# asmirnou/watsor

Measured on NVIDIA H100. Metric: aggregate detection FPS on synthetic 640x480 streams, higher is better.
Workload: dtype f32

## Files before the change

### watsor_b200/csrc/kernels_fused.cu

```cuda
#include <algorithm>
#include <cstdlib>
#include <cstring>

#include "kernels_tc.cuh"
#include "tc_common.cuh"

namespace {

constexpr int F_TH = 8, F_TW = 16;

__device__ __forceinline__ void tma_load_4d(uint32_t dst, const CUtensorMap* map, uint32_t bar, int c0, int c1, int c2,
                                            int c3) {
  asm volatile(
      "cp.async.bulk.tensor.4d.shared::cluster.global.mbarrier::complete_tx::bytes [%0], [%1, {%3, %4, %5, %6}], [%2];" ::
          "r"(dst),
      "l"(map), "r"(bar), "r"(c0), "r"(c1), "r"(c2), "r"(c3)
      : "memory");
}

struct FusedArgs {
  const float* dw_w;
  const float* dw_scale;
  const float* dw_offset;
  const float* scale;
  const float* offset;
  float* out;
  int dw_act, act;
  int C, S, pad_t, pad_l;
  int OH, OW, n_img;
  int N, n_pad, block_n, k_blocks;
  int tiles_x, tiles_y;
  int stages, halo_stages;
  int th_in, tw_in;
};

constexpr int F_CONSUMER_WARPS = 8;
constexpr int F_PRODUCER_WARPS = 8;
constexpr int F_FIRST_PRODUCER_THREAD = 32 * F_CONSUMER_WARPS;
constexpr int F_TMA_WARP = F_CONSUMER_WARPS + F_PRODUCER_WARPS;
constexpr int F_THREADS = F_FIRST_PRODUCER_THREAD + 32 * F_PRODUCER_WARPS + 32;

__device__ __forceinline__ void f_wg_bar_sync(int wg) { asm volatile("bar.sync %0, 128;" ::"r"(2 + wg) : "memory"); }

template <int S, int BN>
__global__ void __launch_bounds__(F_THREADS, 1)
    k_dwpw_tc_x3(const __grid_constant__ CUtensorMap map_in, const __grid_constant__ CUtensorMap map_b,
                 const __grid_constant__ CUtensorMap map_b_lo, FusedArgs g) {
  extern __shared__ __align__(1024) uint8_t smem_raw[];
  uint8_t* smem = reinterpret_cast<uint8_t*>((reinterpret_cast<uintptr_t>(smem_raw) + 1023) & ~(uintptr_t)1023);
  const int halo_bytes = ((g.th_in * g.tw_in * ROW_BYTES + 1023) / 1024) * 1024;
  constexpr int B_TILE_BYTES = BN * ROW_BYTES;
  constexpr int AB_BYTES = 2 * A_TILE_BYTES + 2 * B_TILE_BYTES;
  uint8_t* halo0 = smem;
  uint8_t* ab0 = halo0 + (size_t)g.halo_stages * halo_bytes;
  uint64_t* halo_full = reinterpret_cast<uint64_t*>(ab0 + (size_t)g.stages * AB_BYTES);
  uint64_t* halo_empty = halo_full + g.halo_stages;
  uint64_t* b_full = halo_empty + g.halo_stages;
  uint64_t* a_ready = b_full + g.stages;
  uint64_t* empty = a_ready + g.stages;
  float* s_dw = reinterpret_cast<float*>((reinterpret_cast<uintptr_t>(empty + g.stages) + 15) & ~(uintptr_t)15);

  const int warp = threadIdx.x >> 5, lane = threadIdx.x & 31;
  const int tiles_per_img = g.tiles_x * g.tiles_y;
  const int num_tiles = tiles_per_img * g.n_img;

  if (threadIdx.x == 0) {
    for (int h = 0; h < g.halo_stages; ++h) {
      mbar_init(smem_u32(&halo_full[h]), 1);
      mbar_init(smem_u32(&halo_empty[h]), F_PRODUCER_WARPS);
    }
    for (int s = 0; s < g.stages; ++s) {
      mbar_init(smem_u32(&b_full[s]), 1);
      mbar_init(smem_u32(&a_ready[s]), F_PRODUCER_WARPS);
      mbar_init(smem_u32(&empty[s]), 2);
    }
    fence_barrier_init();
  }
  for (int i = threadIdx.x; i < 9 * g.C; i += blockDim.x) s_dw[i] = g.dw_w[i];
  for (int i = threadIdx.x; i < g.C; i += blockDim.x) {
    s_dw[9 * g.C + i] = g.dw_scale[i];
    s_dw[10 * g.C + i] = g.dw_offset[i];
  }
  float* s_pw = s_dw + 11 * g.C;
  for (int i = threadIdx.x; i < BN; i += blockDim.x) {
    s_pw[i] = i < g.n_pad ? g.scale[i] : 1.f;
    s_pw[BN + i] = i < g.n_pad ? g.offset[i] : 0.f;
  }
  __syncthreads();

  if (warp == F_TMA_WARP) {
    if (elect_one()) {
      int it = 0;
      for (int t = blockIdx.x; t < num_tiles; t += gridDim.x) {
        const int img = t / tiles_per_img, r = t - img * tiles_per_img;
        const int oy0 = (r / g.tiles_x) * F_TH, ox0 = (r % g.tiles_x) * F_TW;
        for (int kb = 0; kb < g.k_blocks; ++kb, ++it) {
          const int h = it % g.halo_stages, s = it % g.stages;
          mbar_wait(smem_u32(&halo_empty[h]), ((it / g.halo_stages) & 1) ^ 1);
          const uint32_t hb = smem_u32(&halo_full[h]);
          mbar_expect_tx(hb, (uint32_t)(g.th_in * g.tw_in * ROW_BYTES));
          tma_load_4d(smem_u32(halo0 + (size_t)h * halo_bytes), &map_in, hb, kb * 32, ox0 * S - g.pad_l,
                      oy0 * S - g.pad_t, img);
          mbar_wait(smem_u32(&empty[s]), ((it / g.stages) & 1) ^ 1);
          const uint32_t bb = smem_u32(&b_full[s]);
          uint8_t* sb = ab0 + (size_t)s * AB_BYTES + 2 * A_TILE_BYTES;
          mbar_expect_tx(bb, 2 * B_TILE_BYTES);
          tma_load_2d(smem_u32(sb), &map_b, bb, kb * 32, 0);
          tma_load_2d(smem_u32(sb + B_TILE_BYTES), &map_b_lo, bb, kb * 32, 0);
        }
      }
    }
  } else if (warp < F_CONSUMER_WARPS) {
    const int wg = warp >> 2;
    const int row = wg * 64 + (warp & 3) * 16 + (lane >> 2);
    const int col = 2 * (lane & 3);
    int it = 0;
    for (int t = blockIdx.x; t < num_tiles; t += gridDim.x) {
      const int img = t / tiles_per_img, r = t - img * tiles_per_img;
      const int oy0 = (r / g.tiles_x) * F_TH, ox0 = (r % g.tiles_x) * F_TW;
      float acc[BN / 2], part[BN / 2];
#pragma unroll
      for (int i = 0; i < BN / 2; ++i) acc[i] = 0.f;
      for (int kb = 0; kb < g.k_blocks; ++kb, ++it) {
        const int s = it % g.stages;
        const uint32_t ph = (it / g.stages) & 1;
        mbar_wait(smem_u32(&a_ready[s]), ph);
        mbar_wait(smem_u32(&b_full[s]), ph);
        const uint32_t a_hi = smem_u32(ab0 + (size_t)s * AB_BYTES) + (uint32_t)(wg * 64 * ROW_BYTES);
        const uint32_t a_lo = a_hi + A_TILE_BYTES;
        const uint32_t b_hi = smem_u32(ab0 + (size_t)s * AB_BYTES) + 2 * A_TILE_BYTES, b_lo = b_hi + B_TILE_BYTES;
        wg_x3_kblock_sum<BN>(acc, part, a_hi, a_lo, b_hi, b_lo);
        f_wg_bar_sync(wg);
        if ((threadIdx.x & 127) == 0) mbar_arrive(smem_u32(&empty[s]));
      }
#pragma unroll
      for (int h = 0; h < 2; ++h) {
        const int rr = row + 8 * h;
        const int oy = oy0 + rr / F_TW, ox = ox0 + rr % F_TW;
        if (oy >= g.OH || ox >= g.OW) continue;
        float* op = g.out + (((size_t)img * g.OH + oy) * g.OW + ox) * g.N;
#pragma unroll
        for (int j = 0; j < BN / 8; ++j) {
          const int c = 8 * j + col;
          if (c >= g.N) break;
          float y0 = affine_rn(acc[4 * j + 2 * h], s_pw[c], s_pw[BN + c]);
          float y1 = affine_rn(acc[4 * j + 2 * h + 1], s_pw[c + 1], s_pw[BN + c + 1]);
          if (g.act == WB_ACT_RELU6) {
            y0 = relu6f(y0);
            y1 = relu6f(y1);
          }
          *reinterpret_cast<float2*>(op + c) = make_float2(y0, y1);
        }
      }
    }
  } else {
    const int pt = threadIdx.x - F_FIRST_PRODUCER_THREAD;
    const int q = pt & 7, slot = pt >> 3;
    int it = 0;
    for (int t = blockIdx.x; t < num_tiles; t += gridDim.x) {
      for (int kb = 0; kb < g.k_blocks; ++kb, ++it) {
        const int h = it % g.halo_stages, s = it % g.stages;
        const int cch = kb * 32 + q * 4;
        float4 wr[9];
#pragma unroll
        for (int k = 0; k < 9; ++k) wr[k] = lds128(smem_u32(s_dw + k * g.C + cch));
        const float4 sc = lds128(smem_u32(s_dw + 9 * g.C + cch));
        const float4 of = lds128(smem_u32(s_dw + 10 * g.C + cch));
        mbar_wait(smem_u32(&halo_full[h]), (it / g.halo_stages) & 1);
        mbar_wait(smem_u32(&empty[s]), ((it / g.stages) & 1) ^ 1);
        const uint32_t hal = smem_u32(halo0 + (size_t)h * halo_bytes);
        const uint32_t a_hi = smem_u32(ab0 + (size_t)s * AB_BYTES);
        const uint32_t a_lo = a_hi + A_TILE_BYTES;
        static_assert(S == 1 && F_PRODUCER_WARPS == 8 && F_TW == 16 && F_TH == 8, "producer mapping");
        constexpr int TW_IN = F_TW + 2;
        const int ty = slot >> 2, x0 = (slot & 3) * 4;
        const uint32_t win = hal + (uint32_t)((ty * TW_IN + x0) * 128 + q * 16);
        float4 acc[4];
#pragma unroll
        for (int o = 0; o < 4; ++o) acc[o] = make_float4(0.f, 0.f, 0.f, 0.f);
#pragma unroll
        for (int ky = 0; ky < 3; ++ky)
#pragma unroll
          for (int c = 0; c < 6; ++c) {
            const float4 x = lds128(win + (uint32_t)((ky * TW_IN + c) * 128));
#pragma unroll
            for (int kx = 0; kx < 3; ++kx) {
              const int o = c - kx;
              if (o >= 0 && o < 4) {
                const float4 ww = wr[ky * 3 + kx];
                acc[o].x = fmaf(x.x, ww.x, acc[o].x);
                acc[o].y = fmaf(x.y, ww.y, acc[o].y);
                acc[o].z = fmaf(x.z, ww.z, acc[o].z);
                acc[o].w = fmaf(x.w, ww.w, acc[o].w);
              }
            }
          }
#pragma unroll
        for (int o = 0; o < 4; ++o) {
          const int r = ty * F_TW + x0 + o;
          float v[4] = {affine_rn(acc[o].x, sc.x, of.x), affine_rn(acc[o].y, sc.y, of.y),
                        affine_rn(acc[o].z, sc.z, of.z), affine_rn(acc[o].w, sc.w, of.w)};
          uint4 hi, lo;
          uint32_t* hp = &hi.x;
          uint32_t* lp = &lo.x;
#pragma unroll
          for (int e = 0; e < 4; ++e) {
            const float a = g.dw_act == WB_ACT_RELU6 ? relu6f(v[e]) : v[e];
            const uint32_t hb = __float_as_uint(a) & 0xFFFFE000u;
            hp[e] = hb;
            lp[e] = __float_as_uint(__fsub_rn(a, __uint_as_float(hb))) & 0xFFFFE000u;
          }
          const uint32_t off = (uint32_t)r * 128u + (uint32_t)((q ^ (r & 7)) << 4);
          sts128(a_hi + off, hi);
          sts128(a_lo + off, lo);
        }
        fence_proxy_async();
        __syncwarp();
        if (lane == 0) {
          mbar_arrive(smem_u32(&a_ready[s]));
          mbar_arrive(smem_u32(&halo_empty[h]));
        }
      }
    }
  }
}

struct FusedPlan {
  int block_n, stages, halo_stages, th_in, tw_in, tiles_x, tiles_y;
  size_t smem;
};

bool make_plan(const wb_layer& dw, const wb_layer& pw, FusedPlan* p) {
  p->block_n = pw.n_pad <= 32 ? 32 : 64;
  p->th_in = (F_TH - 1) * dw.stride + 3;
  p->tw_in = (F_TW - 1) * dw.stride + 3;
  p->tiles_x = (dw.out_w + F_TW - 1) / F_TW;
  p->tiles_y = (dw.out_h + F_TH - 1) / F_TH;
  const size_t halo = ((size_t)p->th_in * p->tw_in * ROW_BYTES + 1023) / 1024 * 1024;
  const size_t ab = 2 * A_TILE_BYTES + 2 * (size_t)p->block_n * ROW_BYTES;
  const size_t budget = 224 * 1024 - 44 * (size_t)dw.out_c;
  for (int st = 2; st >= 1; --st)
    for (int hs = 3; hs >= 2; --hs) {
      if (hs * halo + st * ab <= budget) {
        p->stages = st;
        p->halo_stages = hs;
        p->smem = hs * halo + st * ab + 1024 + 8 * (2 * hs + 3 * st) + 16 + 44 * (size_t)dw.out_c + 8 * (size_t)p->block_n;
        return true;
      }
    }
  return false;
}


}

bool fused_dwpw_supported(const TcWeights& tw, int pw_layer_index, const wb_layer& dw, const wb_layer& pw, int n) {
  if (tw.mode != TC_TF32X3 || getenv("WB_NO_FUSE") != nullptr) return false;
  if (dw.op != WB_OP_DW || pw.op != WB_OP_PW) return false;
  if (dw.kh != 3 || dw.kw != 3 || dw.stride != 1) return false;
  if (dw.out_c % 32 != 0 || pw.in_c != dw.out_c || pw.n_pad > 64 || pw.out_c % 4 != 0) return false;
  {
    const unsigned long long a0 = dw.in_off, a1 = a0 + (unsigned long long)dw.in_h * dw.in_w * dw.in_c;
    const unsigned long long b0 = pw.out_off, b1 = b0 + (unsigned long long)pw.out_h * pw.out_w * pw.out_c;
    if (a0 < b1 && b0 < a1) return false;
  }
  if (!tw.layers[pw_layer_index].ready) return false;
  FusedPlan p;
  if (!make_plan(dw, pw, &p)) return false;
  int dev = 0, sms = 0;
  cudaGetDevice(&dev);
  cudaDeviceGetAttribute(&sms, cudaDevAttrMultiProcessorCount, dev);
  return (long)p.tiles_x * p.tiles_y * n >= sms;
}

int fused_launch_dwpw(const LaunchCtx& lc, const TcWeights& tw, int pw_layer_index, int n, const wb_layer& dw,
                      const wb_layer& pw, const void* in, const float* dw_w, const float* dw_scale, const float* dw_offset,
                      const float* scale, const float* offset, void* out, std::string* err) {
  const TcLayerWeights& w = tw.layers[pw_layer_index];
  FusedPlan p;
  if (!make_plan(dw, pw, &p)) {
    *err = "fused depthwise+pointwise: no shared-memory plan";
    return 1;
  }
  FusedArgs g;
  g.dw_w = dw_w;
  g.dw_scale = dw_scale;
  g.dw_offset = dw_offset;
  g.scale = scale;
  g.offset = offset;
  g.dw_act = dw.act;
  g.act = pw.act;
  g.C = dw.out_c;
  g.S = dw.stride;
  g.pad_t = dw.pad_t;
  g.pad_l = dw.pad_l;
  g.OH = dw.out_h;
  g.OW = dw.out_w;
  g.n_img = n;
  g.N = pw.out_c;
  g.n_pad = pw.n_pad;
  g.block_n = p.block_n;
  g.k_blocks = (dw.out_c + 31) / 32;
  g.out = static_cast<float*>(out);
  g.tiles_x = p.tiles_x;
  g.tiles_y = p.tiles_y;
  g.stages = p.stages;
  g.halo_stages = p.halo_stages;
  g.th_in = p.th_in;
  g.tw_in = p.tw_in;
  alignas(64) CUtensorMap map_in, map_b, map_b_lo;
  {
    unsigned long long dims[4] = {(unsigned long long)dw.in_c, dw.in_w, dw.in_h, (unsigned long long)n};
    unsigned long long st[3] = {(unsigned long long)dw.in_c * 4, (unsigned long long)dw.in_w * dw.in_c * 4,
                                (unsigned long long)dw.in_h * dw.in_w * dw.in_c * 4};
    unsigned box[4] = {32, (unsigned)p.tw_in, (unsigned)p.th_in, 1};
    if (!tc_encode_map(&map_in, in, 4, 4, dims, st, box, false, err)) return 1;
  }
  {
    unsigned long long dims[2] = {(unsigned long long)w.k, (unsigned long long)w.n_pad};
    unsigned long long st[1] = {(unsigned long long)w.k * 4};
    unsigned box[2] = {32, (unsigned)p.block_n};
    if (!tc_encode_map(&map_b, w.w, 4, 2, dims, st, box, true, err)) return 1;
    if (!tc_encode_map(&map_b_lo, w.w_lo, 4, 2, dims, st, box, true, err)) return 1;
  }
  static PerDeviceFlag attr_done[2];
  static int ctas = 0;
  if (ctas == 0) {
    int dev = 0;
    cudaGetDevice(&dev);
    cudaDeviceGetAttribute(&ctas, cudaDevAttrMultiProcessorCount, dev);
  }
  const long tiles = (long)p.tiles_x * p.tiles_y * n;
  const dim3 grid((unsigned)std::min<long>(tiles, ctas));
  auto launch = [&](auto kern, PerDeviceFlag& done) {
    if (!done.get()) {
      cudaError_t e = cudaFuncSetAttribute(kern, cudaFuncAttributeMaxDynamicSharedMemorySize, 227 * 1024);
      if (e != cudaSuccess) return e;
      done.set();
    }
    kern<<<grid, F_THREADS, p.smem, lc.stream>>>(map_in, map_b, map_b_lo, g);
    return cudaGetLastError();
  };
  const cudaError_t e = p.block_n == 32 ? launch(k_dwpw_tc_x3<1, 32>, attr_done[0]) : launch(k_dwpw_tc_x3<1, 64>, attr_done[1]);
  if (e != cudaSuccess) {
    *err = std::string("fused depthwise+pointwise launch: ") + cudaGetErrorString(e);
    return 1;
  }
  ++*lc.launch_counter;
  return 0;
}
```

### watsor_b200/csrc/kernels_tc.cuh

```cuda
#pragma once
#include <string>
#include <vector>

#include "common.cuh"

enum TcMode { TC_BF16 = 0, TC_TF32X1 = 1, TC_TF32X3 = 2 };

struct TcLayerWeights {
  void* w = nullptr;
  void* w_lo = nullptr;
  int n_pad = 0, k = 0, block_n = 0;
  bool ready = false;
  alignas(64) unsigned char tmap_b[128];
  alignas(64) unsigned char tmap_b_lo[128];
};

struct TcWeights {
  int mode = TC_BF16;
  std::vector<TcLayerWeights> layers;
};

bool tc_layer_supported(const wb_layer& L);
int tc_prepare_weights(const std::vector<wb_layer>& layers, const std::vector<wb_tensor_entry>& tensors,
                       const float* host_data, int mode, TcWeights* out, std::string* err);
void tc_free_weights(TcWeights* w);
int tc_launch_gemm(const LaunchCtx& lc, const TcWeights& tw, int layer_index, int n, const wb_layer& L, const void* in,
                   const float* scale, const float* offset, void* out, float* enc, float* logits, int num_anchors,
                   int num_classes_p1, float* partial, size_t partial_floats, int* tile_counters, const void* residual,
                   std::string* err);

bool tc_encode_map(void* map, const void* base, int elem_bytes, int rank, const unsigned long long* dims,
                   const unsigned long long* strides_bytes, const unsigned* box, bool swizzle128, std::string* err,
                   const unsigned* elem_strides = nullptr);

bool fused_dwpw_supported(const TcWeights& tw, int pw_layer_index, const wb_layer& dw, const wb_layer& pw, int n);
int fused_launch_dwpw(const LaunchCtx& lc, const TcWeights& tw, int pw_layer_index, int n, const wb_layer& dw,
                      const wb_layer& pw, const void* in, const float* dw_w, const float* dw_scale, const float* dw_offset,
                      const float* scale, const float* offset, void* out, std::string* err);
```

### watsor_b200/csrc/wb_api.cu

```cuda
#include <dlfcn.h>
#include <nccl.h>

#include <cstdio>
#include <cstdlib>
#include <cstring>
#include <memory>
#include <mutex>
#include <string>
#include <vector>

#include "common.cuh"
#include "kernels_tc.cuh"

#define WB_MAX_CAMERAS 256
#define WB_SLOTS 6

static thread_local std::string g_err;
static int fail(const std::string& msg) {
  g_err = msg;
  return 1;
}
#define CK(call)                                                                              \
  do {                                                                                        \
    cudaError_t e_ = (call);                                                                  \
// ... 293 lines not shown

int wb_set_camera(wb_ctx* c, int cam, int width, int height, int n_zones, const uint8_t* raster, int n_filters,
                  const wb_class_filter* filters, uint32_t cam_flags) {
  REQUIRE(c, "NULL ctx");
  REQUIRE(cam >= 0 && cam < WB_MAX_CAMERAS, "cam_id out of range (0..255)");
  REQUIRE(width > 0 && height > 0, "bad frame size");
  REQUIRE(n_zones >= 0 && n_zones <= WB_MAX_CAMERA_ZONES, "a mask may hold at most 32 zones");
  REQUIRE(n_zones == 0 || raster != nullptr, "zone_raster is NULL");
  REQUIRE(n_filters == 0 || filters != nullptr, "filters is NULL");
  std::lock_guard<std::mutex> lock(c->mu);
  CK(cudaSetDevice(c->device));
  CK(cudaDeviceSynchronize());
  CameraCfg cfg;
  memset(&cfg, 0, sizeof(cfg));
  cfg.width = width;
  cfg.height = height;
  c->max_src_w = std::max(c->max_src_w, width);
  cfg.n_zones = n_zones;
  cfg.has_mask = raster != nullptr ? 1 : 0;
  cfg.check_label = (cam_flags & WB_CAM_NO_LABEL_CHECK) ? 0 : 1;
  for (int i = 0; i < n_filters; ++i) {
    const wb_class_filter& f = filters[i];
    if (f.label == -1) {
      cfg.default_present = 1;
      cfg.default_conf = f.confidence;
      cfg.default_area = f.area;
      cfg.default_has_zone_list = f.has_zone_list ? 1 : 0;
      cfg.default_zone_bits = f.zone_bits;
      continue;
    }
    REQUIRE(f.label >= 0 && f.label < WB_MAX_LABELS, "filter label out of range (0..127)");
    cfg.present[f.label] = 1;
    cfg.conf[f.label] = f.confidence;
    cfg.area[f.label] = f.area;
    cfg.has_zone_list[f.label] = f.has_zone_list ? 1 : 0;
    cfg.zone_bits[f.label] = f.zone_bits;
  }
  if (c->cam_sat[cam]) {
    CK(cudaFree(c->cam_sat[cam]));
    c->cam_sat[cam] = nullptr;
  }
  if (n_zones > 0) {
    size_t sat_elems = (size_t)n_zones * (height + 1) * (width + 1);
    CK(cudaMalloc(&c->cam_sat[cam], sat_elems * sizeof(int32_t)));
    uint8_t* d_r = nullptr;
    size_t rb = (size_t)n_zones * height * width;
    CK(cudaMalloc(&d_r, rb));
    CK(cudaMemcpy(d_r, raster, rb, cudaMemcpyHostToDevice));
    int lcnt = 0;
    LaunchCtx lc{c->slots[0].stream, &lcnt};
    launch_build_sat(lc, d_r, n_zones, height, width, c->cam_sat[cam]);
    CK(cudaGetLastError());
    CK(cudaStreamSynchronize(c->slots[0].stream));
    CK(cudaFree(d_r));
    cfg.sat = c->cam_sat[cam];
  }
  c->h_cams[cam] = cfg;
  CK(cudaMemcpy(c->d_cams + cam, &cfg, sizeof(cfg), cudaMemcpyHostToDevice));
  return 0;
}

int wb_register_host(wb_ctx* c, void* ptr, size_t bytes) {
  REQUIRE(c && ptr && bytes, "NULL argument");
  std::lock_guard<std::mutex> lock(c->mu);
  CK(cudaSetDevice(c->device));
  CK(cudaHostRegister(ptr, bytes, cudaHostRegisterDefault));
  c->registered.push_back(ptr);
  return 0;
}
int wb_unregister_host(wb_ctx* c, void* ptr) {
  REQUIRE(c && ptr, "NULL argument");
  std::lock_guard<std::mutex> lock(c->mu);
  for (size_t i = 0; i < c->registered.size(); ++i)
    if (c->registered[i] == ptr) {
      CK(cudaHostUnregister(ptr));
      c->registered.erase(c->registered.begin() + i);
      return 0;
    }
  return fail("pointer was not registered");
}

}

template <typename T>
static int run_layers(wb_ctx* c, Slot& s, cudaStream_t st, int n, const float* pre, int first_layer,
                      int last_layer) {
  LaunchCtx lc{st, &s.launches};
  T* arena = static_cast<T*>(s.arena);
  const int NA = c->hdr.num_anchors, C1 = c->hdr.num_classes + 1;
  const size_t end = last_layer < 0 ? c->layers.size() : (size_t)last_layer + 1;
  for (size_t li = (size_t)first_layer; li < end; ++li) {
    const wb_layer& L = c->layers[li];
    const T* in = arena + (size_t)L.in_off * n;
    const T* in2 = arena + (size_t)L.in2_off * n;
    T* outp = arena + (size_t)L.out_off * n;
    const float* w = L.w_tensor >= 0 ? c->tensor(L.w_tensor) : nullptr;
    const float* sc = L.scale_tensor >= 0 ? c->tensor(L.scale_tensor) : nullptr;
    const float* of = L.offset_tensor >= 0 ? c->tensor(L.offset_tensor) : nullptr;
    switch (L.op) {
      case WB_OP_STEM:
        launch_stem<T>(lc, s.d_desc, pre, n, L, c->hdr.input_h, c->hdr.input_w, c->hdr.pre_mul, c->hdr.pre_sub, w,
                       sc, of, outp, c->max_src_w);
        break;
      case WB_OP_DW: {
        if (c->precision == 2 && li + 1 < end) {
          const wb_layer& P = c->layers[li + 1];
          if (P.in_off == L.out_off && fused_dwpw_supported(c->tc, (int)li + 1, L, P, n)) {
            std::string err;
            if (fused_launch_dwpw(lc, c->tc, (int)li + 1, n, L, P, static_cast<const void*>(in), w, sc, of,
                                  c->tensor(P.scale_tensor), c->tensor(P.offset_tensor),
                                  static_cast<void*>(arena + (size_t)P.out_off * n), &err))
              return fail("layers " + std::string(L.name) + " + " + P.name + ": " + err);
            ++li;
            break;
          }
        }
        launch_dw<T>(lc, n, L, in, w, sc, of, outp);
        break;
      }
      case WB_OP_ADD:
        launch_add<T>(lc, (size_t)n * L.out_h * L.out_w * L.out_c, in, in2, outp);
        break;
      case WB_OP_MAXPOOL:
      case WB_OP_AVGPOOL:
        launch_pool<T>(lc, n, L, in, outp);
        break;
      case WB_OP_COPY:
        launch_copy_channels<T>(lc, n, L, in, outp);
        break;
      case WB_OP_PW:
      case WB_OP_CONV:
      case WB_OP_HEAD:
        if (c->precision != 0 && tc_layer_supported(L)) {
          const void* residual = nullptr;
          void* dst = static_cast<void*>(outp);
          bool fuse_add = false;
          if (c->precision != 1 && L.op == WB_OP_PW && L.act == WB_ACT_NONE && li + 1 < end && getenv("WB_NO_FUSE_ADD") == nullptr) {
            const wb_layer& A = c->layers[li + 1];
            const unsigned long long a0 = L.in_off, a1 = a0 + (unsigned long long)L.in_h * L.in_w * L.in_c;
            const unsigned long long b0 = A.out_off, b1 = b0 + (unsigned long long)A.out_h * A.out_w * A.out_c;
            if (A.op == WB_OP_ADD && (A.in_off == L.out_off || A.in2_off == L.out_off) && A.in_off != A.in2_off &&
                !(a0 < b1 && b0 < a1)) {
              const uint32_t other = A.in_off == L.out_off ? A.in2_off : A.in_off;
              residual = static_cast<const void*>(arena + (size_t)other * n);
              dst = static_cast<void*>(arena + (size_t)A.out_off * n);
              fuse_add = true;
            }
          }
          std::string err;
          if (tc_launch_gemm(lc, c->tc, (int)li, n, L, static_cast<const void*>(in), sc, of, dst, s.d_enc, s.d_logits, NA,
                             C1, s.d_partial, s.partial_floats, s.d_tile_counters, residual, &err))
            return fail("layer " + std::string(L.name) + ": " + err);
          if (fuse_add) ++li;
        } else {
          launch_gemm_cc<T>(lc, n, L, in, w, sc, of, outp, s.d_enc, s.d_logits, NA, C1, s.d_partial, s.partial_floats);
        }
        break;
      default:
        return fail("unknown layer op " + std::to_string(L.op));
    }
  }
  CK(cudaGetLastError());
  return 0;
}

static int run_post(wb_ctx* c, Slot& s, cudaStream_t st, int n, uint32_t flags, bool want_raw = false) {
  LaunchCtx lc{st, &s.launches};
  float* rb = want_raw ? s.d_raw : nullptr;
  float* rs = want_raw ? rb + (size_t)c->max_batch * WB_MAX_DETECTIONS * 4 : nullptr;
  float* rc = want_raw ? rs + (size_t)c->max_batch * WB_MAX_DETECTIONS : nullptr;
  launch_post(lc, n, c->pp, s.d_enc, s.d_logits, c->tensor(c->hdr.anchors_tensor), s.d_desc, c->d_cams, flags,
              s.d_dec, s.d_cand_count, s.d_cand, s.d_sel_count, s.d_sel, s.d_out, s.d_verdicts, rb, rs, rc,
              want_raw ? s.d_raw_num : nullptr, s.d_kept_hist);
  CK(cudaGetLastError());
  return 0;
}

static int run_all(wb_ctx* c, Slot& s, cudaStream_t st, int n, uint32_t flags) {
  int rc = c->precision == 1 ? run_layers<__nv_bfloat16>(c, s, st, n, nullptr, 0, -1)
                             : run_layers<float>(c, s, st, n, nullptr, 0, -1);
  if (rc) return rc;
  return run_post(c, s, st, n, flags);
}

static int enqueue_kernels(wb_ctx* c, Slot& s, cudaStream_t st, int n, uint32_t flags) {
  const uint32_t gflags = flags & WB_F_FUSE_FILTERS;
  if (!c->use_graph) {
    s.launches = 0;
    return run_all(c, s, st, n, gflags);
  }
  if (s.graph_exec == nullptr || s.graph_n != n || s.graph_flags != gflags || s.graph_src_w != c->max_src_w) {
    if (s.graph_exec) {
      cudaGraphExecDestroy(s.graph_exec);
      s.graph_exec = nullptr;
    }
    s.launches = 0;
    if (int rc = run_all(c, s, st, n, gflags)) return rc;
    CK(cudaStreamSynchronize(st));
    cudaGraph_t graph = nullptr;
    CK(cudaStreamBeginCapture(st, cudaStreamCaptureModeThreadLocal));
    s.launches = 0;
    int rc = run_all(c, s, st, n, gflags);
    cudaError_t e = cudaStreamEndCapture(st, &graph);
    if (rc) return rc;
    if (e != cudaSuccess) return fail(std::string("cudaStreamEndCapture: ") + cudaGetErrorString(e));
    CK(cudaGraphInstantiate(&s.graph_exec, graph, 0));
    CK(cudaGraphDestroy(graph));
    s.graph_n = n;
    s.graph_flags = gflags;
    s.graph_src_w = c->max_src_w;
  }
  CK(cudaGraphLaunch(s.graph_exec, st));
  return 0;
}

static int frame_format(uint32_t flags, int* fmt) {
  REQUIRE(!((flags & WB_F_YUV420P) && (flags & WB_F_NV12)), "WB_F_YUV420P and WB_F_NV12 are mutually exclusive");
  *fmt = (flags & WB_F_YUV420P) ? WB_FMT_YUV420P : (flags & WB_F_NV12) ? WB_FMT_NV12 : WB_FMT_RGB24;
  return 0;
}

static int fill_desc(wb_ctx* c, Slot& s, int n, const uint8_t* const* frames, const int32_t* cam_ids,
                     bool on_device, int fmt, cudaStream_t st) {
  size_t total = 0;
  for (int i = 0; i < n; ++i) {
    int cam = cam_ids[i];
    REQUIRE(cam >= 0 && cam < WB_MAX_CAMERAS && c->h_cams[cam].width > 0,
            "cam_id " + std::to_string(cam) + " has not been configured with wb_set_camera");
    REQUIRE(frames == nullptr || frames[i] != nullptr, "NULL frame pointer");
    const CameraCfg& cc = c->h_cams[cam];
// ... 200 lines not shown
  c->last_launches = s.launches;
  return 0;
}

int wb_postprocess(wb_ctx* c, int n, const float* enc, const float* logits, const int32_t* cam_ids, uint32_t flags,
                   wb_detection* const* out, uint32_t* const* verdicts, float* boxes, float* scores, float* classes,
                   int32_t* num) {
  REQUIRE(c && enc && logits && cam_ids, "NULL argument");
  REQUIRE(n >= 1 && n <= c->max_batch, "batch size out of range");
  std::lock_guard<std::mutex> lock(c->mu);
  CK(cudaSetDevice(c->device));
  Slot& s = c->slots[0];
  REQUIRE(!s.busy, "slot 0 is busy");
  cudaStream_t st = c->stream_of(0);
  const int NA = c->hdr.num_anchors, C1 = c->hdr.num_classes + 1;
  CK(cudaMemcpyAsync(s.d_enc, enc, sizeof(float) * (size_t)n * NA * 4, cudaMemcpyHostToDevice, st));
  CK(cudaMemcpyAsync(s.d_logits, logits, sizeof(float) * (size_t)n * NA * C1, cudaMemcpyHostToDevice, st));
  if (int rc = fill_desc(c, s, n, nullptr, cam_ids, false, WB_FMT_RGB24, st)) return rc;
  s.launches = 0;
  if (int rc = run_post(c, s, st, n, flags, true)) return rc;
  const size_t B = c->max_batch;
  CK(cudaMemcpyAsync(s.h_out, s.d_out, sizeof(wb_detection) * (size_t)n * WB_MAX_DETECTIONS, cudaMemcpyDeviceToHost, st));
  CK(cudaMemcpyAsync(s.h_verdicts, s.d_verdicts, sizeof(uint32_t) * (size_t)n * WB_MAX_DETECTIONS, cudaMemcpyDeviceToHost, st));
  CK(cudaMemcpyAsync(s.h_raw, s.d_raw, sizeof(float) * B * WB_MAX_DETECTIONS * 6, cudaMemcpyDeviceToHost, st));
  CK(cudaMemcpyAsync(s.h_raw_num, s.d_raw_num, sizeof(int) * n, cudaMemcpyDeviceToHost, st));
  CK(cudaStreamSynchronize(st));
  for (int i = 0; i < n; ++i) {
    if (out && out[i]) memcpy(out[i], s.h_out + (size_t)i * WB_MAX_DETECTIONS, sizeof(wb_detection) * WB_MAX_DETECTIONS);
    if (verdicts && verdicts[i])
      memcpy(verdicts[i], s.h_verdicts + (size_t)i * WB_MAX_DETECTIONS, sizeof(uint32_t) * WB_MAX_DETECTIONS);
  }
  if (boxes) memcpy(boxes, s.h_raw, sizeof(float) * (size_t)n * WB_MAX_DETECTIONS * 4);
  if (scores) memcpy(scores, s.h_raw + B * WB_MAX_DETECTIONS * 4, sizeof(float) * (size_t)n * WB_MAX_DETECTIONS);
  if (classes) memcpy(classes, s.h_raw + B * WB_MAX_DETECTIONS * 5, sizeof(float) * (size_t)n * WB_MAX_DETECTIONS);
  if (num) memcpy(num, s.h_raw_num, sizeof(int) * n);
  c->last_launches = s.launches;
  return 0;
}

int wb_filter_rows(wb_ctx* c, int cam, int n_rows, wb_detection* rows, uint32_t* verdicts) {
  REQUIRE(c && rows && verdicts, "NULL argument");
  REQUIRE(n_rows >= 1 && n_rows <= c->frows_cap, "n_rows out of range");
  std::lock_guard<std::mutex> lock(c->mu);
  REQUIRE(cam >= 0 && cam < WB_MAX_CAMERAS && c->h_cams[cam].width > 0, "camera has not been configured");
  CK(cudaSetDevice(c->device));
  cudaStream_t st = c->fstream;
  CK(cudaMemcpyAsync(c->d_frows, rows, sizeof(wb_detection) * n_rows, cudaMemcpyHostToDevice, st));
  int launches = 0;
  LaunchCtx lc{st, &launches};
  launch_filter_rows(lc, c->d_cams + cam, n_rows, c->d_frows, c->d_fverd);
  CK(cudaGetLastError());
  CK(cudaMemcpyAsync(rows, c->d_frows, sizeof(wb_detection) * n_rows, cudaMemcpyDeviceToHost, st));
  CK(cudaMemcpyAsync(verdicts, c->d_fverd, sizeof(uint32_t) * n_rows, cudaMemcpyDeviceToHost, st));
  CK(cudaStreamSynchronize(st));
  return 0;
}

int wb_last_launch_count(wb_ctx* c, int* launches) {
  REQUIRE(c && launches, "NULL argument");
  *launches = c->last_launches;
  return 0;
}

int wb_profile_layers(wb_ctx* c, int n, const uint8_t* const* device_frames, const int32_t* cam_ids,
                      float* ms, int32_t* kinds, int max_launches, int* n_out) {
  REQUIRE(c && device_frames && cam_ids && ms && kinds && n_out, "NULL argument");
  REQUIRE(n >= 1 && n <= c->max_batch, "batch size out of range");
  std::lock_guard<std::mutex> lock(c->mu);
  CK(cudaSetDevice(c->device));
  Slot& s = c->slots[0];
  REQUIRE(!s.busy, "slot 0 is busy");
  cudaStream_t st = c->stream_of(0);
  if (int rc = fill_desc(c, s, n, device_frames, cam_ids, true, WB_FMT_RGB24, st)) return rc;
  const int nl = (int)c->layers.size();
  REQUIRE(max_launches >= nl + 1, "max_launches too small");
  std::vector<cudaEvent_t> ev(nl + 2);
  for (auto& e : ev) CK(cudaEventCreate(&e));
  const int REPS = 10;
  s.launches = 0;
  if (int rc = run_all(c, s, st, n, 0)) return rc;
  s.launches = 0;
  CK(cudaEventRecord(ev[0], st));
  for (int li = 0; li < nl; ++li) {
    int last = li;
    if (c->precision == 2 && li + 1 < nl && c->layers[li].op == WB_OP_DW &&
        c->layers[li + 1].in_off == c->layers[li].out_off &&
        fused_dwpw_supported(c->tc, li + 1, c->layers[li], c->layers[li + 1], n))
      last = li + 1;
    if (last == li && c->precision != 0 && c->precision != 1 && li + 1 < nl && c->layers[li].op == WB_OP_PW &&
        c->layers[li].act == WB_ACT_NONE && c->layers[li + 1].op == WB_OP_ADD && tc_layer_supported(c->layers[li]) &&
        (c->layers[li + 1].in_off == c->layers[li].out_off || c->layers[li + 1].in2_off == c->layers[li].out_off) &&
        getenv("WB_NO_FUSE_ADD") == nullptr)
      last = li + 1;
    const int first = li;
    const bool time_on_first = last != li && c->layers[li].op == WB_OP_PW;
    if (last != li && !time_on_first) {
      CK(cudaEventRecord(ev[li + 1], st));
      kinds[li] = (int)c->layers[li].op;
      ++li;
    }
    for (int r = 0; r < REPS; ++r) {
      int rc = c->precision == 1 ? run_layers<__nv_bfloat16>(c, s, st, n, nullptr, first, last)
                                 : run_layers<float>(c, s, st, n, nullptr, first, last);
      if (rc) return rc;
    }
    CK(cudaEventRecord(ev[li + 1], st));
    kinds[li] = (int)c->layers[li].op;
    if (time_on_first) {
      ++li;
      CK(cudaEventRecord(ev[li + 1], st));
      kinds[li] = (int)c->layers[li].op;
    }
  }
  for (int r = 0; r < REPS; ++r)
    if (int rc = run_post(c, s, st, n, 0)) return rc;
  CK(cudaEventRecord(ev[nl + 1], st));
  CK(cudaEventSynchronize(ev[nl + 1]));
  for (int li = 0; li <= nl; ++li) {
    CK(cudaEventElapsedTime(&ms[li], ev[li], ev[li + 1]));
    ms[li] /= REPS;
  }
  s.launches /= REPS;
  kinds[nl] = 100;
  for (auto& e : ev) cudaEventDestroy(e);
  *n_out = nl + 1;
  c->last_launches = s.launches;
  return 0;
}

}

namespace {
struct NcclApi {
  void* handle = nullptr;
  ncclResult_t (*GetUniqueId)(ncclUniqueId*) = nullptr;
  ncclResult_t (*CommInitRank)(ncclComm_t*, int, ncclUniqueId, int) = nullptr;
  ncclResult_t (*CommDestroy)(ncclComm_t) = nullptr;
  ncclResult_t (*GroupStart)() = nullptr;
  ncclResult_t (*GroupEnd)() = nullptr;
  ncclResult_t (*Send)(const void*, size_t, ncclDataType_t, int, ncclComm_t, cudaStream_t) = nullptr;
  ncclResult_t (*Recv)(void*, size_t, ncclDataType_t, int, ncclComm_t, cudaStream_t) = nullptr;
  const char* (*GetErrorString)(ncclResult_t) = nullptr;
  std::string error;
};

NcclApi* nccl_api() {
  static NcclApi api;
  static std::once_flag once;
  std::call_once(once, [] {
    api.handle = dlopen("libnccl.so.2", RTLD_NOW | RTLD_NOLOAD);
    const char* override_path = getenv("WB_NCCL_LIB");
    if (!api.handle && override_path && override_path[0]) api.handle = dlopen(override_path, RTLD_NOW | RTLD_GLOBAL);
    if (!api.handle) api.handle = dlopen("libnccl.so.2", RTLD_NOW | RTLD_GLOBAL);
    if (!api.handle) api.handle = dlopen("libnccl.so", RTLD_NOW | RTLD_GLOBAL);
    if (!api.handle) {
      const char* e = dlerror();
      api.error = std::string("cannot load NCCL (libnccl.so.2): ") + (e ? e : "not found");
      return;
    }
    bool ok = true;
    auto sym = [&](const char* name) {
      void* p = dlsym(api.handle, name);
      if (!p) {
        ok = false;
        api.error = std::string("NCCL symbol missing: ") + name;
      }
      return p;
    };
    api.GetUniqueId = reinterpret_cast<decltype(api.GetUniqueId)>(sym("ncclGetUniqueId"));
    api.CommInitRank = reinterpret_cast<decltype(api.CommInitRank)>(sym("ncclCommInitRank"));
    api.CommDestroy = reinterpret_cast<decltype(api.CommDestroy)>(sym("ncclCommDestroy"));
    api.GroupStart = reinterpret_cast<decltype(api.GroupStart)>(sym("ncclGroupStart"));
    api.GroupEnd = reinterpret_cast<decltype(api.GroupEnd)>(sym("ncclGroupEnd"));
    api.Send = reinterpret_cast<decltype(api.Send)>(sym("ncclSend"));
    api.Recv = reinterpret_cast<decltype(api.Recv)>(sym("ncclRecv"));
    api.GetErrorString = reinterpret_cast<decltype(api.GetErrorString)>(sym("ncclGetErrorString"));
    if (!ok) api.handle = nullptr;
  });
  return &api;
}
}

#define NCCL_CK(api, call)                                                                      \
  do {                                                                                          \
    ncclResult_t _r = (call);                                                                   \
    if (_r != ncclSuccess) return fail(std::string(#call) + ": " + (api)->GetErrorString(_r));  \
  } while (0)

static_assert(sizeof(ncclUniqueId) == WB_COMM_ID_BYTES, "ncclUniqueId is 128 bytes");

int wb_comm_unique_id(uint8_t* id_out) {
// ... 79 lines not shown
```

### watsor_b200/model.py

```python
import struct
from dataclasses import dataclass, field
from typing import List

import numpy as np

from .graphdef import GraphDef

MAGIC = b'WB200M01'
OP_STEM, OP_DW, OP_PW, OP_CONV, OP_ADD, OP_HEAD, OP_MAXPOOL, OP_AVGPOOL, OP_COPY = 1, 2, 3, 4, 5, 6, 7, 8, 9
OP_NAMES = {1: 'stem', 2: 'dw', 3: 'pw', 4: 'conv', 5: 'add', 6: 'head', 7: 'maxpool', 8: 'avgpool', 9: 'copy'}
ACT_NONE, ACT_RELU6 = 0, 1
HEADER_BYTES, LAYER_BYTES, TENSOR_BYTES = 256, 128, 16
N_ALIGN = 16
ARENA_ALIGN = 256


def same_pad(in_size, k, s):
    out = -(-in_size // s)
    total = max((out - 1) * s + k - in_size, 0)
    return out, total // 2


@dataclass
class Layer:
    op: int
    act: int = ACT_NONE
    in_h: int = 0
    in_w: int = 0
    in_c: int = 0
    out_h: int = 0
    out_w: int = 0
    out_c: int = 0
    kh: int = 1
    kw: int = 1
    stride: int = 1
    pad_t: int = 0
    pad_l: int = 0
    in_off: int = 0
    in2_off: int = 0
    out_off: int = 0
    w_tensor: int = -1
    scale_tensor: int = -1
    offset_tensor: int = -1
    n_pad: int = 0
    anchors_per_loc: int = 0
    row_off: int = 0
    n_box: int = 0
    n_cls: int = 0
    name: str = ''
    src: str = ''
    src2: str = ''
    dst: str = ''

    @property
    def macs(self):
        if self.op == OP_DW:
            return self.out_h * self.out_w * self.out_c * self.kh * self.kw
        if self.op in (OP_ADD, OP_MAXPOOL, OP_AVGPOOL, OP_COPY):
            return 0
        return self.out_h * self.out_w * self.out_c * self.kh * self.kw * self.in_c


@dataclass
class Model:
    input_h: int = 300
    input_w: int = 300
    num_classes: int = 0
    num_anchors: int = 0
    pre_mul: float = 0.0
    pre_sub: float = 0.0
    scale_y: float = 10.0
    scale_x: float = 10.0
    scale_h: float = 5.0
    scale_w: float = 5.0
    logit_scale: float = 1.0
    iou_thr: float = 0.6
    score_thr: float = 0.3
    max_per_class: int = 100
    max_total: int = 100
    class_offset: float = 1.0
    arena_elems: int = 0
    anchors_tensor: int = -1
    layers: List[Layer] = field(default_factory=list)
    tensors: List[np.ndarray] = field(default_factory=list)
    name: str = ''

    def add_tensor(self, arr):
        self.tensors.append(np.ascontiguousarray(arr, dtype=np.float32))
        return len(self.tensors) - 1

    @property
    def anchors(self):
        return self.tensors[self.anchors_tensor].reshape(-1, 4)

    @property
    def macs_per_frame(self):
        return sum(l.macs for l in self.layers)

    def plan_arena(self):
        last_use = {}
        for i, l in enumerate(self.layers):
            for t in (l.src, l.src2):
                if t:
                    last_use[t] = i
        for i, l in enumerate(self.layers[:-1]):
            nxt = self.layers[i + 1]
            if l.op == OP_DW and nxt.op == OP_PW and nxt.src == l.dst and l.src:
                last_use[l.src] = max(last_use[l.src], i + 1)
        for i, l in enumerate(self.layers[:-1]):
            nxt = self.layers[i + 1]
            if l.op == OP_PW and nxt.op == OP_ADD and l.dst in (nxt.src, nxt.src2) and l.src:
                last_use[l.src] = max(last_use[l.src], i + 1)
        for i, l in enumerate(self.layers[:-2]):
            d, p_ = self.layers[i + 1], self.layers[i + 2]
            if l.op == OP_PW and d.op == OP_DW and p_.op == OP_PW and d.src == l.dst and p_.src == d.dst and l.src:
                end_ = i + 2
                if i + 3 < len(self.layers) and self.layers[i + 3].op == OP_ADD and \
                        p_.dst in (self.layers[i + 3].src, self.layers[i + 3].src2):
                    end_ = i + 3
                last_use[l.src] = max(last_use[l.src], end_)
        size = {}
        for l in self.layers:
            if l.dst:
                size[l.dst] = -(-(l.out_h * l.out_w * l.out_c) // ARENA_ALIGN) * ARENA_ALIGN
        free = []
        top = 0
        where = {}

        def alloc(n):
            nonlocal top
            for k, (o, s) in enumerate(free):
                if s >= n:
                    if s == n:
                        free.pop(k)
                    else:
                        free[k] = (o + n, s - n)
                    return o
            o = top
            top += n
            return o

        def release(o, n):
            free.append((o, n))
            free.sort()
            merged = []
            for o2, s2 in free:
                if merged and merged[-1][0] + merged[-1][1] == o2:
                    merged[-1] = (merged[-1][0], merged[-1][1] + s2)
                else:
                    merged.append((o2, s2))
            free[:] = merged

        for i, l in enumerate(self.layers):
            if l.dst:
                if l.dst not in where:
                    where[l.dst] = alloc(size[l.dst])
                l.out_off = where[l.dst]
            if l.src and l.src in where:
                l.in_off = where[l.src]
            if l.src2 and l.src2 in where:
                l.in2_off = where[l.src2]
            for t in [t for t, lu in last_use.items() if lu == i and t in where]:
                release(where[t], size[t])
        self.arena_elems = top

    def to_blob(self):
        hdr = struct.pack(
            '<8sIIIIIIfffffffffIIfIIQ', MAGIC, len(self.layers), len(self.tensors), self.input_h,
            self.input_w, self.num_classes, self.num_anchors, self.pre_mul, self.pre_sub,
            self.scale_y, self.scale_x, self.scale_h, self.scale_w, self.logit_scale, self.iou_thr,
            self.score_thr, self.max_per_class, self.max_total, self.class_offset,
            self.anchors_tensor, 0, self.arena_elems)
        hdr = hdr.ljust(HEADER_BYTES, b'\0')
        out = [hdr]
        for l in self.layers:
            rec = struct.pack(
                '<IIIIIIIIIIIIIIIIiiiIIIII', l.op, l.act, l.in_h, l.in_w, l.in_c, l.out_h, l.out_w,
                l.out_c, l.kh, l.kw, l.stride, l.pad_t, l.pad_l, l.in_off, l.in2_off, l.out_off,
                l.w_tensor, l.scale_tensor, l.offset_tensor, l.n_pad, l.anchors_per_loc, l.row_off,
                l.n_box, l.n_cls)
            name = l.name.encode()[:LAYER_BYTES - len(rec) - 1]
            out.append((rec + name).ljust(LAYER_BYTES, b'\0'))
        off = 0
        for t in self.tensors:
            out.append(struct.pack('<QQ', off, t.size))
            off += -(-t.size // 64) * 64
        for t in self.tensors:
            pad = -(-t.size // 64) * 64 - t.size
            out.append(t.tobytes())
            if pad:
                out.append(b'\0' * (4 * pad))
        return b''.join(out)

    @staticmethod
    def from_blob(blob):
        m = Model()
        f = struct.unpack_from('<8sIIIIIIfffffffffIIfIIQ', blob, 0)
        assert f[0] == MAGIC, 'not a WB200 model blob'
        (n_layers, n_tensors, m.input_h, m.input_w, m.num_classes, m.num_anchors, m.pre_mul,
         m.pre_sub, m.scale_y, m.scale_x, m.scale_h, m.scale_w, m.logit_scale, m.iou_thr,
         m.score_thr, m.max_per_class, m.max_total, m.class_offset, m.anchors_tensor, _,
         m.arena_elems) = f[1:]
        pos = HEADER_BYTES
# ... 539 lines not shown
```

Baseline: 12280.

## Extend fused depthwise+pointwise kernel to stride 2, padded channels, and residual add

Generalizes the fused dw3x3+pw tensor-core kernel so it also handles stride-2 depthwise layers and channel counts that are not multiples of 32, padding the smem weight tables with zeros. It also adds an optional residual input to the epilogue, so a following ADD layer is folded in. Span selection is factored into a shared helper, and the SM-count occupancy check is replaced by a minimum spatial size. The aim is to cut launches and intermediate tensor round-trips through global memory, at the risk of running fused tiles on layers where the fused pipeline underuses the GPU.

```diff
diff --git a/watsor_b200/csrc/kernels_fused.cu b/watsor_b200/csrc/kernels_fused.cu
--- a/watsor_b200/csrc/kernels_fused.cu
+++ b/watsor_b200/csrc/kernels_fused.cu
@@ -25,6 +25,7 @@
   const float* scale;
   const float* offset;
   float* out;
+  const float* residual;
   int dw_act, act;
   int C, S, pad_t, pad_l;
   int OH, OW, n_img;
@@ -76,12 +77,16 @@
     }
     fence_barrier_init();
   }
-  for (int i = threadIdx.x; i < 9 * g.C; i += blockDim.x) s_dw[i] = g.dw_w[i];
-  for (int i = threadIdx.x; i < g.C; i += blockDim.x) {
-    s_dw[9 * g.C + i] = g.dw_scale[i];
-    s_dw[10 * g.C + i] = g.dw_offset[i];
-  }
-  float* s_pw = s_dw + 11 * g.C;
+  const int cs = g.k_blocks * 32;
+  for (int i = threadIdx.x; i < 9 * cs; i += blockDim.x) {
+    const int k = i / cs, ch = i - k * cs;
+    s_dw[i] = ch < g.C ? g.dw_w[k * g.C + ch] : 0.f;
+  }
+  for (int i = threadIdx.x; i < cs; i += blockDim.x) {
+    s_dw[9 * cs + i] = i < g.C ? g.dw_scale[i] : 0.f;
+    s_dw[10 * cs + i] = i < g.C ? g.dw_offset[i] : 0.f;
+  }
+  float* s_pw = s_dw + 11 * cs;
   for (int i = threadIdx.x; i < BN; i += blockDim.x) {
     s_pw[i] = i < g.n_pad ? g.scale[i] : 1.f;
     s_pw[BN + i] = i < g.n_pad ? g.offset[i] : 0.f;
@@ -138,7 +143,8 @@
         const int rr = row + 8 * h;
         const int oy = oy0 + rr / F_TW, ox = ox0 + rr % F_TW;
         if (oy >= g.OH || ox >= g.OW) continue;
-        float* op = g.out + (((size_t)img * g.OH + oy) * g.OW + ox) * g.N;
+        const size_t po = (((size_t)img * g.OH + oy) * g.OW + ox) * g.N;
+        float* op = g.out + po;
 #pragma unroll
         for (int j = 0; j < BN / 8; ++j) {
           const int c = 8 * j + col;
@@ -149,6 +155,11 @@
             y0 = relu6f(y0);
             y1 = relu6f(y1);
           }
+          if (g.residual != nullptr) {
+            const float2 r2 = *reinterpret_cast<const float2*>(g.residual + po + c);
+            y0 = __fadd_rn(y0, r2.x);
+            y1 = __fadd_rn(y1, r2.y);
+          }
           *reinterpret_cast<float2*>(op + c) = make_float2(y0, y1);
         }
       }
@@ -163,30 +174,30 @@
         const int cch = kb * 32 + q * 4;
         float4 wr[9];
 #pragma unroll
-        for (int k = 0; k < 9; ++k) wr[k] = lds128(smem_u32(s_dw + k * g.C + cch));
-        const float4 sc = lds128(smem_u32(s_dw + 9 * g.C + cch));
-        const float4 of = lds128(smem_u32(s_dw + 10 * g.C + cch));
+        for (int k = 0; k < 9; ++k) wr[k] = lds128(smem_u32(s_dw + k * cs + cch));
+        const float4 sc = lds128(smem_u32(s_dw + 9 * cs + cch));
+        const float4 of = lds128(smem_u32(s_dw + 10 * cs + cch));
         mbar_wait(smem_u32(&halo_full[h]), (it / g.halo_stages) & 1);
         mbar_wait(smem_u32(&empty[s]), ((it / g.stages) & 1) ^ 1);
         const uint32_t hal = smem_u32(halo0 + (size_t)h * halo_bytes);
         const uint32_t a_hi = smem_u32(ab0 + (size_t)s * AB_BYTES);
         const uint32_t a_lo = a_hi + A_TILE_BYTES;
-        static_assert(S == 1 && F_PRODUCER_WARPS == 8 && F_TW == 16 && F_TH == 8, "producer mapping");
-        constexpr int TW_IN = F_TW + 2;
+        static_assert((S == 1 || S == 2) && F_PRODUCER_WARPS == 8 && F_TW == 16 && F_TH == 8, "producer mapping");
+        constexpr int TW_IN = (F_TW - 1) * S + 3, NC = 3 * S + 3;
         const int ty = slot >> 2, x0 = (slot & 3) * 4;
-        const uint32_t win = hal + (uint32_t)((ty * TW_IN + x0) * 128 + q * 16);
+        const uint32_t win = hal + (uint32_t)((ty * S * TW_IN + x0 * S) * 128 + q * 16);
         float4 acc[4];
 #pragma unroll
         for (int o = 0; o < 4; ++o) acc[o] = make_float4(0.f, 0.f, 0.f, 0.f);
 #pragma unroll
         for (int ky = 0; ky < 3; ++ky)
 #pragma unroll
-          for (int c = 0; c < 6; ++c) {
+          for (int c = 0; c < NC; ++c) {
             const float4 x = lds128(win + (uint32_t)((ky * TW_IN + c) * 128));
 #pragma unroll
             for (int kx = 0; kx < 3; ++kx) {
-              const int o = c - kx;
-              if (o >= 0 && o < 4) {
+              const int o = (c - kx) / S;
+              if (c >= kx && (c - kx) % S == 0 && o < 4) {
                 const float4 ww = wr[ky * 3 + kx];
                 acc[o].x = fmaf(x.x, ww.x, acc[o].x);
                 acc[o].y = fmaf(x.y, ww.y, acc[o].y);
@@ -238,13 +249,14 @@
   p->tiles_y = (dw.out_h + F_TH - 1) / F_TH;
   const size_t halo = ((size_t)p->th_in * p->tw_in * ROW_BYTES + 1023) / 1024 * 1024;
   const size_t ab = 2 * A_TILE_BYTES + 2 * (size_t)p->block_n * ROW_BYTES;
-  const size_t budget = 224 * 1024 - 44 * (size_t)dw.out_c;
+  const size_t dw_bytes = 44 * (size_t)((dw.out_c + 31) / 32 * 32);
+  const size_t budget = 224 * 1024 - dw_bytes;
   for (int st = 2; st >= 1; --st)
     for (int hs = 3; hs >= 2; --hs) {
       if (hs * halo + st * ab <= budget) {
         p->stages = st;
         p->halo_stages = hs;
-        p->smem = hs * halo + st * ab + 1024 + 8 * (2 * hs + 3 * st) + 16 + 44 * (size_t)dw.out_c + 8 * (size_t)p->block_n;
+        p->smem = hs * halo + st * ab + 1024 + 8 * (2 * hs + 3 * st) + 16 + dw_bytes + 8 * (size_t)p->block_n;
         return true;
       }
     }
@@ -254,28 +266,21 @@
 
 }
 
-bool fused_dwpw_supported(const TcWeights& tw, int pw_layer_index, const wb_layer& dw, const wb_layer& pw, int n) {
-  if (tw.mode != TC_TF32X3 || getenv("WB_NO_FUSE") != nullptr) return false;
+bool fused_dwpw_supported(const TcWeights& tw, int pw_layer_index, const wb_layer& dw, const wb_layer& pw) {
+  if (tw.mode != TC_TF32X3) return false;
   if (dw.op != WB_OP_DW || pw.op != WB_OP_PW) return false;
-  if (dw.kh != 3 || dw.kw != 3 || dw.stride != 1) return false;
-  if (dw.out_c % 32 != 0 || pw.in_c != dw.out_c || pw.n_pad > 64 || pw.out_c % 4 != 0) return false;
-  {
-    const unsigned long long a0 = dw.in_off, a1 = a0 + (unsigned long long)dw.in_h * dw.in_w * dw.in_c;
-    const unsigned long long b0 = pw.out_off, b1 = b0 + (unsigned long long)pw.out_h * pw.out_w * pw.out_c;
-    if (a0 < b1 && b0 < a1) return false;
-  }
+  if (dw.kh != 3 || dw.kw != 3 || (dw.stride != 1 && dw.stride != 2)) return false;
+  if (dw.out_h * dw.out_w < 32 * 32) return false;
+  if (dw.out_c % 4 != 0 || (dw.out_c + 31) / 32 >= 16 || pw.in_c != dw.out_c || pw.n_pad > 64 || pw.out_c % 4 != 0)
+    return false;
   if (!tw.layers[pw_layer_index].ready) return false;
   FusedPlan p;
-  if (!make_plan(dw, pw, &p)) return false;
-  int dev = 0, sms = 0;
-  cudaGetDevice(&dev);
-  cudaDeviceGetAttribute(&sms, cudaDevAttrMultiProcessorCount, dev);
-  return (long)p.tiles_x * p.tiles_y * n >= sms;
+  return make_plan(dw, pw, &p);
 }
 
 int fused_launch_dwpw(const LaunchCtx& lc, const TcWeights& tw, int pw_layer_index, int n, const wb_layer& dw,
                       const wb_layer& pw, const void* in, const float* dw_w, const float* dw_scale, const float* dw_offset,
-                      const float* scale, const float* offset, void* out, std::string* err) {
+                      const float* scale, const float* offset, const float* residual, void* out, std::string* err) {
   const TcLayerWeights& w = tw.layers[pw_layer_index];
   FusedPlan p;
   if (!make_plan(dw, pw, &p)) {
@@ -302,6 +307,7 @@
   g.block_n = p.block_n;
   g.k_blocks = (dw.out_c + 31) / 32;
   g.out = static_cast<float*>(out);
+  g.residual = residual;
   g.tiles_x = p.tiles_x;
   g.tiles_y = p.tiles_y;
   g.stages = p.stages;
@@ -323,7 +329,7 @@
     if (!tc_encode_map(&map_b, w.w, 4, 2, dims, st, box, true, err)) return 1;
     if (!tc_encode_map(&map_b_lo, w.w_lo, 4, 2, dims, st, box, true, err)) return 1;
   }
-  static PerDeviceFlag attr_done[2];
+  static PerDeviceFlag attr_done[4];
   static int ctas = 0;
   if (ctas == 0) {
     int dev = 0;
@@ -341,7 +347,11 @@
     kern<<<grid, F_THREADS, p.smem, lc.stream>>>(map_in, map_b, map_b_lo, g);
     return cudaGetLastError();
   };
-  const cudaError_t e = p.block_n == 32 ? launch(k_dwpw_tc_x3<1, 32>, attr_done[0]) : launch(k_dwpw_tc_x3<1, 64>, attr_done[1]);
+  const int ki = (dw.stride == 2 ? 2 : 0) + (p.block_n == 32 ? 0 : 1);
+  const cudaError_t e = ki == 0   ? launch(k_dwpw_tc_x3<1, 32>, attr_done[0])
+                        : ki == 1 ? launch(k_dwpw_tc_x3<1, 64>, attr_done[1])
+                        : ki == 2 ? launch(k_dwpw_tc_x3<2, 32>, attr_done[2])
+                                  : launch(k_dwpw_tc_x3<2, 64>, attr_done[3]);
   if (e != cudaSuccess) {
     *err = std::string("fused depthwise+pointwise launch: ") + cudaGetErrorString(e);
     return 1;
diff --git a/watsor_b200/csrc/kernels_tc.cuh b/watsor_b200/csrc/kernels_tc.cuh
--- a/watsor_b200/csrc/kernels_tc.cuh
+++ b/watsor_b200/csrc/kernels_tc.cuh
@@ -33,7 +33,7 @@
                    const unsigned long long* strides_bytes, const unsigned* box, bool swizzle128, std::string* err,
                    const unsigned* elem_strides = nullptr);
 
-bool fused_dwpw_supported(const TcWeights& tw, int pw_layer_index, const wb_layer& dw, const wb_layer& pw, int n);
+bool fused_dwpw_supported(const TcWeights& tw, int pw_layer_index, const wb_layer& dw, const wb_layer& pw);
 int fused_launch_dwpw(const LaunchCtx& lc, const TcWeights& tw, int pw_layer_index, int n, const wb_layer& dw,
                       const wb_layer& pw, const void* in, const float* dw_w, const float* dw_scale, const float* dw_offset,
-                      const float* scale, const float* offset, void* out, std::string* err);
+                      const float* scale, const float* offset, const float* residual, void* out, std::string* err);
diff --git a/watsor_b200/csrc/wb_api.cu b/watsor_b200/csrc/wb_api.cu
--- a/watsor_b200/csrc/wb_api.cu
+++ b/watsor_b200/csrc/wb_api.cu
@@ -399,6 +399,48 @@
 
 }
 
+enum SpanKind {
+  SPAN_ONE,
+  SPAN_DW_PW,
+  SPAN_DW_PW_ADD,
+  SPAN_PW_ADD,
+};
+struct Span {
+  size_t last;
+  SpanKind kind;
+};
+
+static bool arena_disjoint(const wb_layer& reader, const wb_layer& writer) {
+  const unsigned long long a0 = reader.in_off, a1 = a0 + (unsigned long long)reader.in_h * reader.in_w * reader.in_c;
+  const unsigned long long b0 = writer.out_off, b1 = b0 + (unsigned long long)writer.out_h * writer.out_w * writer.out_c;
+  return !(a0 < b1 && b0 < a1);
+}
+
+static Span fused_span(const wb_ctx* c, size_t li, size_t end) {
+  const std::vector<wb_layer>& Ls = c->layers;
+  const wb_layer& L = Ls[li];
+  auto residual_add_after = [&](size_t p) {
+    if (c->precision == 0 || c->precision == 1 || p + 1 >= end || getenv("WB_NO_FUSE_ADD") != nullptr) return false;
+    const wb_layer& P = Ls[p], &A = Ls[p + 1];
+    return P.op == WB_OP_PW && P.act == WB_ACT_NONE && A.op == WB_OP_ADD &&
+           (A.in_off == P.out_off || A.in2_off == P.out_off) && A.in_off != A.in2_off;
+  };
+  if (L.op == WB_OP_DW && c->precision == 2 && li + 1 < end && getenv("WB_NO_FUSE") == nullptr) {
+    const wb_layer& P = Ls[li + 1];
+    if (P.in_off == L.out_off && fused_dwpw_supported(c->tc, (int)li + 1, L, P)) {
+      if (residual_add_after(li + 1)) {
+        if (arena_disjoint(L, Ls[li + 2])) return {li + 2, SPAN_DW_PW_ADD};
+      } else if (arena_disjoint(L, P)) {
+        return {li + 1, SPAN_DW_PW};
+      }
+    }
+  }
+  if (L.op == WB_OP_PW && c->precision != 0 && tc_layer_supported(L) && residual_add_after(li) &&
+      arena_disjoint(L, Ls[li + 1]))
+    return {li + 1, SPAN_PW_ADD};
+  return {li, SPAN_ONE};
+}
+
 template <typename T>
 static int run_layers(wb_ctx* c, Slot& s, cudaStream_t st, int n, const float* pre, int first_layer,
                       int last_layer) {
@@ -420,17 +462,20 @@
                        sc, of, outp, c->max_src_w);
         break;
       case WB_OP_DW: {
-        if (c->precision == 2 && li + 1 < end) {
+        const Span sp = fused_span(c, li, end);
+        if (sp.kind == SPAN_DW_PW || sp.kind == SPAN_DW_PW_ADD) {
           const wb_layer& P = c->layers[li + 1];
-          if (P.in_off == L.out_off && fused_dwpw_supported(c->tc, (int)li + 1, L, P, n)) {
-            std::string err;
-            if (fused_launch_dwpw(lc, c->tc, (int)li + 1, n, L, P, static_cast<const void*>(in), w, sc, of,
-                                  c->tensor(P.scale_tensor), c->tensor(P.offset_tensor),
-                                  static_cast<void*>(arena + (size_t)P.out_off * n), &err))
-              return fail("layers " + std::string(L.name) + " + " + P.name + ": " + err);
-            ++li;
-            break;
-          }
+          const wb_layer& O = c->layers[sp.last];
+          const float* residual = nullptr;
+          if (sp.kind == SPAN_DW_PW_ADD)
+            residual = reinterpret_cast<const float*>(arena + (size_t)(O.in_off == P.out_off ? O.in2_off : O.in_off) * n);
+          std::string err;
+          if (fused_launch_dwpw(lc, c->tc, (int)li + 1, n, L, P, static_cast<const void*>(in), w, sc, of,
+                                c->tensor(P.scale_tensor), c->tensor(P.offset_tensor), residual,
+                                static_cast<void*>(arena + (size_t)O.out_off * n), &err))
+            return fail("layers " + std::string(L.name) + " .. " + O.name + ": " + err);
+          li = sp.last;
+          break;
         }
         launch_dw<T>(lc, n, L, in, w, sc, of, outp);
         break;
@@ -451,18 +496,12 @@
         if (c->precision != 0 && tc_layer_supported(L)) {
           const void* residual = nullptr;
           void* dst = static_cast<void*>(outp);
-          bool fuse_add = false;
-          if (c->precision != 1 && L.op == WB_OP_PW && L.act == WB_ACT_NONE && li + 1 < end && getenv("WB_NO_FUSE_ADD") == nullptr) {
+          const bool fuse_add = fused_span(c, li, end).kind == SPAN_PW_ADD;
+          if (fuse_add) {
             const wb_layer& A = c->layers[li + 1];
-            const unsigned long long a0 = L.in_off, a1 = a0 + (unsigned long long)L.in_h * L.in_w * L.in_c;
-            const unsigned long long b0 = A.out_off, b1 = b0 + (unsigned long long)A.out_h * A.out_w * A.out_c;
-            if (A.op == WB_OP_ADD && (A.in_off == L.out_off || A.in2_off == L.out_off) && A.in_off != A.in2_off &&
-                !(a0 < b1 && b0 < a1)) {
-              const uint32_t other = A.in_off == L.out_off ? A.in2_off : A.in_off;
-              residual = static_cast<const void*>(arena + (size_t)other * n);
-              dst = static_cast<void*>(arena + (size_t)A.out_off * n);
-              fuse_add = true;
-            }
+            const uint32_t other = A.in_off == L.out_off ? A.in2_off : A.in_off;
+            residual = static_cast<const void*>(arena + (size_t)other * n);
+            dst = static_cast<void*>(arena + (size_t)A.out_off * n);
           }
           std::string err;
           if (tc_launch_gemm(lc, c->tc, (int)li, n, L, static_cast<const void*>(in), sc, of, dst, s.d_enc, s.d_logits, NA,
@@ -829,22 +868,12 @@
   s.launches = 0;
   CK(cudaEventRecord(ev[0], st));
   for (int li = 0; li < nl; ++li) {
-    int last = li;
-    if (c->precision == 2 && li + 1 < nl && c->layers[li].op == WB_OP_DW &&
-        c->layers[li + 1].in_off == c->layers[li].out_off &&
-        fused_dwpw_supported(c->tc, li + 1, c->layers[li], c->layers[li + 1], n))
-      last = li + 1;
-    if (last == li && c->precision != 0 && c->precision != 1 && li + 1 < nl && c->layers[li].op == WB_OP_PW &&
-        c->layers[li].act == WB_ACT_NONE && c->layers[li + 1].op == WB_OP_ADD && tc_layer_supported(c->layers[li]) &&
-        (c->layers[li + 1].in_off == c->layers[li].out_off || c->layers[li + 1].in2_off == c->layers[li].out_off) &&
-        getenv("WB_NO_FUSE_ADD") == nullptr)
-      last = li + 1;
-    const int first = li;
-    const bool time_on_first = last != li && c->layers[li].op == WB_OP_PW;
-    if (last != li && !time_on_first) {
+    const Span sp = fused_span(c, li, nl);
+    const int first = li, last = (int)sp.last;
+    const int timed = sp.kind == SPAN_DW_PW || sp.kind == SPAN_DW_PW_ADD ? li + 1 : li;
+    for (; li < timed; ++li) {
       CK(cudaEventRecord(ev[li + 1], st));
       kinds[li] = (int)c->layers[li].op;
-      ++li;
     }
     for (int r = 0; r < REPS; ++r) {
       int rc = c->precision == 1 ? run_layers<__nv_bfloat16>(c, s, st, n, nullptr, first, last)
@@ -853,7 +882,7 @@
     }
     CK(cudaEventRecord(ev[li + 1], st));
     kinds[li] = (int)c->layers[li].op;
-    if (time_on_first) {
+    while (li < last) {
       ++li;
       CK(cudaEventRecord(ev[li + 1], st));
       kinds[li] = (int)c->layers[li].op;
diff --git a/watsor_b200/model.py b/watsor_b200/model.py
--- a/watsor_b200/model.py
+++ b/watsor_b200/model.py
@@ -106,19 +106,15 @@
         for i, l in enumerate(self.layers[:-1]):
             nxt = self.layers[i + 1]
             if l.op == OP_DW and nxt.op == OP_PW and nxt.src == l.dst and l.src:
-                last_use[l.src] = max(last_use[l.src], i + 1)
+                end_ = i + 1
+                if i + 2 < len(self.layers) and self.layers[i + 2].op == OP_ADD and \
+                        nxt.dst in (self.layers[i + 2].src, self.layers[i + 2].src2):
+                    end_ = i + 2
+                last_use[l.src] = max(last_use[l.src], end_)
         for i, l in enumerate(self.layers[:-1]):
             nxt = self.layers[i + 1]
             if l.op == OP_PW and nxt.op == OP_ADD and l.dst in (nxt.src, nxt.src2) and l.src:
                 last_use[l.src] = max(last_use[l.src], i + 1)
-        for i, l in enumerate(self.layers[:-2]):
-            d, p_ = self.layers[i + 1], self.layers[i + 2]
-            if l.op == OP_PW and d.op == OP_DW and p_.op == OP_PW and d.src == l.dst and p_.src == d.dst and l.src:
-                end_ = i + 2
-                if i + 3 < len(self.layers) and self.layers[i + 3].op == OP_ADD and \
-                        p_.dst in (self.layers[i + 3].src, self.layers[i + 3].src2):
-                    end_ = i + 3
-                last_use[l.src] = max(last_use[l.src], end_)
         size = {}
         for l in self.layers:
             if l.dst:
```

Measured after the change: 12850 (median of 6 runs). 4.7% higher.
